# suous/RecNeXt

Measured on AMD Instinct MI355X. Metric: images/sec RecNeXt-M3 224x224 bf16, higher is better.
Workload: dtype bf16

## Files before the change

### recnext_amd/csrc/rcx_mlp.hip

```cpp
#include "rcx_common.h"
#include "rcx_launch.h"
#include "rcx_gelu.h"
#include <type_traits>

#ifdef RCX_MLP_STAMPS
#define RCX_MLP_STAMP(k)                                                                                        \
    {                                                                                                           \
        __builtin_amdgcn_sched_barrier(0);                                                                      \
        unsigned long long t_;                                                                                  \
        asm volatile("s_memtime %0\n\ts_waitcnt lgkmcnt(0)" : "=s"(t_)::"memory");                              \
        __builtin_amdgcn_sched_barrier(0);                                                                      \
        tsum[k] += t_ - tlast;                                                                                  \
        tlast = t_;                                                                                             \
    }
#define RCX_MLP_STAMP_BEGIN                                                                                     \
    unsigned long long tsum[7] = {0, 0, 0, 0, 0, 0, 0}, tlast;                                                  \
    asm volatile("s_memtime %0\n\ts_waitcnt lgkmcnt(0)" : "=s"(tlast)::"memory");
#define RCX_MLP_STAMP_STEP tsum[6] += 1;
#define RCX_MLP_STAMP_END(slot)                                                                                 \
    if (stamps && (threadIdx.x & 63) == 0) {                                                                    \
        _Pragma("unroll") for (int k_ = 0; k_ < 7; ++k_) stamps[(size_t)(slot) * 8 + k_] = tsum[k_];            \
    }
#define RCX_MLP_STAMP_PARM , unsigned long long (&tsum)[7], unsigned long long& tlast
#define RCX_MLP_STAMP_PASS , tsum, tlast
#define RCX_MLP_STAMP_ARG , unsigned long long* __restrict__ stamps
#define RCX_MLP_STAMP_VAL , g_stamps
namespace rcx {
static unsigned long long* g_stamps = nullptr;
}
#else
#define RCX_MLP_STAMP(k)
#define RCX_MLP_STAMP_BEGIN
#define RCX_MLP_STAMP_STEP
#define RCX_MLP_STAMP_END(slot)
#define RCX_MLP_STAMP_PARM
#define RCX_MLP_STAMP_PASS
#define RCX_MLP_STAMP_ARG
#define RCX_MLP_STAMP_VAL
#endif

#ifndef RCX_MLP_PINNED
#define RCX_MLP_PINNED true
#endif

namespace rcx {
namespace mlp {

typedef float f32x16 __attribute__((ext_vector_type(16)));
typedef float f32x4q __attribute__((ext_vector_type(4)));
typedef float f32x2q __attribute__((ext_vector_type(2)));
typedef __bf16 bf16x8 __attribute__((ext_vector_type(8)));
typedef __bf16 bf16x4 __attribute__((ext_vector_type(4)));
typedef unsigned u32x4q __attribute__((ext_vector_type(4)));
typedef unsigned u32x2q __attribute__((ext_vector_type(2)));

__device__ __forceinline__ void wave_sync()
{
    __builtin_amdgcn_fence(__ATOMIC_RELEASE, "wavefront");
    __builtin_amdgcn_wave_barrier();
    __builtin_amdgcn_fence(__ATOMIC_ACQUIRE, "wavefront");
}


__device__ __forceinline__ __amdgpu_buffer_rsrc_t token_rows(const void* p, unsigned nbytes) { return __builtin_amdgcn_make_buffer_rsrc((void*)p, 0, nbytes, 0x00020000); }

#define RCX_MLP_ZERO(D, N)                                                                                                                \
    _Pragma("unroll") for (int n_ = 0; n_ < N; ++n_) _Pragma("unroll") for (int i_ = 0; i_ < 16; ++i_) D[n_][i_] = 0.f;

#define RCX_MLP_STAGE_Z(ZA)                                                                                                               \
    _Pragma("unroll") for (int q = 0; q < ZH; ++q) {                                                                                      \
        _Pragma("unroll") for (int i = 0; i < KH; ++i) *reinterpret_cast<u32x4q*>(Lt + (ZA)) = zq[q * KH + i];                            \
        wave_sync();                                                                                                                      \
        _Pragma("unroll") for (int k = 0; k < KH; ++k)                                                                                    \
            zb[q * KH + k] = __builtin_bit_cast(bf16x8, *reinterpret_cast<const u32x4q*>(Lt + r * ZP + 32 * k + 16 * h));                 \
        wave_sync();                                                                                                                      \
    }

#define RCX_MLP_IMAGE_QUAD(D2, B2, DST)                                                                                                   \
    {                                                                                                                                     \
        const f32x4q bb = *reinterpret_cast<const f32x4q*>(B2);                                                                           \
        *reinterpret_cast<f32x4q*>(DST) = f32x4q{D2[4 * g] + bb.x, D2[4 * g + 1] + bb.y, D2[4 * g + 2] + bb.z, D2[4 * g + 3] + bb.w};     \
    }

__device__ __forceinline__ bf16x8 rows_plus_x(f32x4q lo, f32x4q hi, u32x4q xv)
{
    bf16x8 o;
    o[0] = (__bf16)(lo.x + __uint_as_float(xv.x << 16)); o[1] = (__bf16)(lo.y + __uint_as_float(xv.x & 0xffff0000u));
    o[2] = (__bf16)(lo.z + __uint_as_float(xv.y << 16)); o[3] = (__bf16)(lo.w + __uint_as_float(xv.y & 0xffff0000u));
    o[4] = (__bf16)(hi.x + __uint_as_float(xv.z << 16)); o[5] = (__bf16)(hi.y + __uint_as_float(xv.z & 0xffff0000u));
    o[6] = (__bf16)(hi.z + __uint_as_float(xv.w << 16)); o[7] = (__bf16)(hi.w + __uint_as_float(xv.w & 0xffff0000u));
    return o;
}

constexpr int imax(int a, int b) { return a > b ? a : b; }
constexpr size_t bias_bytes(int HT, int CT) { return sizeof(float) * 32 * (HT + CT); }

template <int KS1, int HT, int CT, int NW, bool STAGED>
struct SmallLds {
    static constexpr int NF = HT * (KS1 + 2 * CT), ZP = 32 * KS1 + 16, OP = 128 * CT + 16, IMG = STAGED ? 32 * imax(ZP, OP) : 0;
    static constexpr size_t b1 = (size_t)NF * 1024, images = b1 + bias_bytes(HT, CT), bytes = images + (size_t)NW * IMG;
};
template <int KS1, int HT, int CT, int NW, int ZH>
struct StreamLds {
    static constexpr int NCH = KS1 + 2 * CT, ZP = 32 * KS1 / ZH + 16, OP = 256 + 16, IMG = 32 * imax(ZP, OP);
    static constexpr size_t b1 = (size_t)2 * NCH * 1024, images = b1 + bias_bytes(HT, CT), bytes = images + (size_t)NW * IMG;
};
template <int KS1, int HT, int CT>
struct PairLds {
    static constexpr int NW = 8, NS = 3, ZH = 4, NCH = KS1 + 2 * CT, ZP = 32 * KS1 / ZH + 16, OP = 128 + 16, IMG = 32 * imax(ZP, OP);
    static constexpr size_t b1 = (size_t)NS * NCH * 1024, images = b1 + bias_bytes(HT, CT), bytes = images + (size_t)NW * IMG;
};
template <int KS1, int HT, int CT>
struct Res128Lds {
    static constexpr int NW = 8, ZH = 4, NCH = KS1 + 2 * CT, NF = HT * NCH, ZP = 32 * KS1 / ZH + 16, OC = 16, OP = 4 * OC + 16, IMG = 32 * imax(ZP, OP);
    static constexpr size_t b1 = (size_t)NF * 1024, images = b1 + bias_bytes(HT, CT), bytes = images + (size_t)NW * IMG;
};
template <int KS1, int HT, int CT, int NW>
struct WideLds {
    static constexpr int ZBYTES = 2 * KS1 * 1024, XBYTES = NW * 4 * 1024, OP = 256 + 16, IMG = 32 * OP;
    static constexpr size_t xchg = ZBYTES, b1 = (size_t)ZBYTES + 2 * XBYTES, bytes = b1 + bias_bytes(HT, CT);
    static_assert(NW * IMG <= ZBYTES + XBYTES, "the output images alias the z fragments and exchange buffer 0");
};

#define RCX_MLP_HIDDEN_GELU(D1, QUAD)                                                                                                     \
    bf16x8 hb[2];                                                                                                                         \
    gelu_f32x2 gv[8];                                                                                                                     \
    _Pragma("unroll") for (int g = 0; g < 4; ++g) {                                                                                       \
        const f32x4q bb = QUAD;                                                                                                           \
        gv[2 * g] = gelu_f32x2{D1[4 * g] + bb.x, D1[4 * g + 1] + bb.y};                                                                   \
        gv[2 * g + 1] = gelu_f32x2{D1[4 * g + 2] + bb.z, D1[4 * g + 3] + bb.w};                                                           \
    }                                                                                                                                     \
    {                                                                                                                                     \
        gelu_f32x2 ga[4] = {gv[0], gv[1], gv[2], gv[3]}, gb[4] = {gv[4], gv[5], gv[6], gv[7]};                                            \
        gelu2x_batch<4>(ga);                                                                                                              \
        gelu2x_batch<4>(gb);                                                                                                              \
        _Pragma("unroll") for (int i = 0; i < 4; ++i) { gv[i] = ga[i]; gv[4 + i] = gb[i]; }                                               \
    }                                                                                                                                     \
    _Pragma("unroll") for (int g = 0; g < 4; ++g) {                                                                                       \
        hb[g >> 1][4 * (g & 1) + 0] = (__bf16)gv[2 * g].x; hb[g >> 1][4 * (g & 1) + 1] = (__bf16)gv[2 * g].y;                             \
        hb[g >> 1][4 * (g & 1) + 2] = (__bf16)gv[2 * g + 1].x; hb[g >> 1][4 * (g & 1) + 3] = (__bf16)gv[2 * g + 1].y;                     \
    }

template <int KS1, int CT, int RD>
__device__ __forceinline__ void hidden_tile_ring(const u32x4q* Lc, const float* b1t, int lane, int h, const bf16x8 (&zb)[KS1], f32x16 (&d2)[CT] RCX_MLP_STAMP_PARM)
{
    constexpr int R1 = KS1 < RD ? KS1 : RD, N2 = 2 * CT, R2 = N2 < RD ? N2 : RD;
    u32x4q ring[RD];
#pragma unroll
    for (int j = 0; j < R1; ++j) ring[j] = Lc[j * 64 + lane];
    RCX_MLP_STAMP(0)
    f32x16 d1;
#pragma unroll
    for (int i = 0; i < 16; ++i) d1[i] = 0.f;
#pragma unroll
    for (int ks = 0; ks < KS1; ++ks) {
        const bf16x8 a = __builtin_bit_cast(bf16x8, ring[ks % R1]);
        if (ks + R1 < KS1) ring[ks % R1] = Lc[(ks + R1) * 64 + lane];
        d1 = __builtin_amdgcn_mfma_f32_32x32x16_bf16(a, zb[ks], d1, 0, 0, 0);
    }
    RCX_MLP_STAMP(1)
#ifndef RCX_MLP_STAMPS
#pragma unroll
    for (int f = 0; f < R2; ++f) ring[f] = Lc[(KS1 + 2 * (f % CT) + f / CT) * 64 + lane];
#endif
    RCX_MLP_HIDDEN_GELU(d1, *reinterpret_cast<const f32x4q*>(b1t + 8 * g + 4 * h))
#ifdef RCX_MLP_STAMPS
#pragma unroll
    for (int f = 0; f < R2; ++f) ring[f] = Lc[(KS1 + 2 * (f % CT) + f / CT) * 64 + lane];
#endif
    RCX_MLP_STAMP(2)
#pragma unroll
    for (int f = 0; f < N2; ++f) {
        const bf16x8 a = __builtin_bit_cast(bf16x8, ring[f % R2]);
        if (f + R2 < N2) ring[f % R2] = Lc[(KS1 + 2 * ((f + R2) % CT) + (f + R2) / CT) * 64 + lane];
        d2[f % CT] = __builtin_amdgcn_mfma_f32_32x32x16_bf16(a, hb[f / CT], d2[f % CT], 0, 0, 0);
    }
    RCX_MLP_STAMP(3)
}

template <int KS1, int CT, int RD, int PRE2, int B1AT>
__device__ __forceinline__ void hidden_tile_pinned(const u32x4q* Lc, const float* b1t, int lane, int h, const bf16x8 (&zb)[KS1], f32x16 (&d2)[CT] RCX_MLP_STAMP_PARM)
{
    constexpr int R1 = KS1 < RD ? KS1 : RD, N2 = 2 * CT, R2 = N2 < RD ? N2 : RD, P2 = PRE2 < R2 ? PRE2 : R2;
    static_assert(B1AT >= 1 && B1AT <= KS1 && P2 >= 1, "b1 is requested inside D1, W2 before the GELU");
    u32x4q ring[RD];
#pragma unroll
    for (int j = 0; j < R1; ++j) ring[j] = Lc[j * 64 + lane];
    RCX_MLP_STAMP(0)
    f32x16 d1;
#pragma unroll
    for (int i = 0; i < 16; ++i) d1[i] = 0.f;
    f32x4q bq[4];
#pragma unroll
    for (int ks = 0; ks < KS1; ++ks) {
        const bf16x8 a = __builtin_bit_cast(bf16x8, ring[ks % R1]);
        if (ks + R1 < KS1) ring[ks % R1] = Lc[(ks + R1) * 64 + lane];
        if (ks == KS1 - B1AT) {
#pragma unroll
            for (int g = 0; g < 4; ++g) bq[g] = *reinterpret_cast<const f32x4q*>(b1t + 8 * g + 4 * h);
        }
        d1 = __builtin_amdgcn_mfma_f32_32x32x16_bf16(a, zb[ks], d1, 0, 0, 0);
        __builtin_amdgcn_sched_barrier(0);
    }
    RCX_MLP_STAMP(1)
#pragma unroll
    for (int f = 0; f < P2; ++f) ring[f] = Lc[(KS1 + 2 * (f % CT) + f / CT) * 64 + lane];
    __builtin_amdgcn_sched_barrier(0);
    RCX_MLP_HIDDEN_GELU(d1, bq[g])
    __builtin_amdgcn_sched_barrier(0);
#pragma unroll
    for (int f = P2; f < R2; ++f) ring[f] = Lc[(KS1 + 2 * (f % CT) + f / CT) * 64 + lane];
    __builtin_amdgcn_sched_barrier(0);
    RCX_MLP_STAMP(2)
#pragma unroll
    for (int f = 0; f < N2; ++f) {
        const bf16x8 a = __builtin_bit_cast(bf16x8, ring[f % R2]);
        if (f + R2 < N2) ring[f % R2] = Lc[(KS1 + 2 * ((f + R2) % CT) + (f + R2) / CT) * 64 + lane];
        d2[f % CT] = __builtin_amdgcn_mfma_f32_32x32x16_bf16(a, hb[f / CT], d2[f % CT], 0, 0, 0);
        __builtin_amdgcn_sched_barrier(0);
    }
    RCX_MLP_STAMP(3)
}

template <int KS1, int HT, int CT, int NW, int WPS, bool KX, bool OX, bool STAGED>
__global__ void __launch_bounds__(64 * NW, WPS)
k_channel_mlp(const bf16_t* __restrict__ z, const bf16_t* __restrict__ xres, bf16_t* __restrict__ y, const u32x4q* __restrict__ wfrag, const float* __restrict__ bias,
              int M, int C, int ntiles RCX_MLP_STAMP_ARG)
{
    extern __shared__ __attribute__((aligned(16))) unsigned char lds_raw[];
    using L = SmallLds<KS1, HT, CT, NW, STAGED>;
    constexpr int NF = L::NF;
    const u32x4q* const Lf = reinterpret_cast<const u32x4q*>(lds_raw);
    const float* const Lb1 = reinterpret_cast<const float*>(lds_raw + L::b1);
    const float* const Lb2 = Lb1 + 32 * HT;
    {
        u32x4q* Lw = reinterpret_cast<u32x4q*>(lds_raw);
        for (int i = threadIdx.x; i < NF * 64; i += 64 * NW) Lw[i] = wfrag[i];
        float* Lb = reinterpret_cast<float*>(lds_raw + L::b1);
        for (int i = threadIdx.x; i < 32 * (HT + CT); i += 64 * NW) Lb[i] = bias[i];
    }
    __syncthreads();
    const int wave = threadIdx.x >> 6, lane = threadIdx.x & 63, r = lane & 31, h = lane >> 5;
    const unsigned nbytes = (unsigned)M * (unsigned)C * 2u;
    const __amdgpu_buffer_rsrc_t zsrc = token_rows(z, nbytes), xsrc = token_rows(xres, nbytes), ysrc = token_rows(y, nbytes);
    unsigned zk[KS1], oc[CT][4];
#pragma unroll
    for (int ks = 0; ks < KS1; ++ks) zk[ks] = KX || 16 * ks + 8 * h < C ? 2u * (16 * ks + 8 * h) : 0x80000000u;
#pragma unroll
    for (int ct = 0; ct < CT; ++ct)
#pragma unroll
        for (int g = 0; g < 4; ++g) oc[ct][g] = OX || 32 * ct + 8 * g + 4 * h < C ? 2u * (32 * ct + 8 * g + 4 * h) : 0x80000000u;

    RCX_MLP_STAMP_BEGIN
    auto hidden_tile = [&](int ht, const bf16x8 (&zb)[KS1], f32x16 (&d2)[CT]) {
        hidden_tile_ring<KS1, CT, 4>(Lf + (size_t)ht * (KS1 + 2 * CT) * 64, Lb1 + 32 * ht, lane, h, zb, d2 RCX_MLP_STAMP_PASS);
        RCX_MLP_STAMP_STEP
    };
    const int stride = gridDim.x * NW;
    int tile = blockIdx.x * NW + wave;
    if constexpr (STAGED) {
        constexpr int ZP = L::ZP, OP = L::OP;
        unsigned char* const Lt = lds_raw + L::images + (size_t)wave * L::IMG;
        const unsigned RB = 2u * (unsigned)C;
        unsigned go[KS1], za[KS1], oa[KS1];
        bool live[KS1];
#pragma unroll
        for (int i = 0; i < KS1; ++i) {
            const unsigned o = 1024u * i + 16u * lane, t = o / RB, bb = o - t * RB;
            live[i] = o < 32u * RB;
            go[i] = live[i] ? o : 0x80000000u;
            za[i] = t * ZP + bb;
            oa[i] = t * OP + 2u * bb;
        }
        u32x4q zq[KS1];
        auto load_z = [&](int t) {
#pragma unroll
            for (int i = 0; i < KS1; ++i) zq[i] = __builtin_bit_cast(u32x4q, __builtin_amdgcn_raw_buffer_load_b128(zsrc, (int)((unsigned)t * 32u * RB + go[i]), 0, 0));
        };
        if (tile < ntiles) load_z(tile);
        for (; tile < ntiles; tile += stride) {
            const unsigned base = (unsigned)tile * 32u * RB;
#pragma unroll
            for (int i = 0; i < KS1; ++i)
                if (live[i]) *reinterpret_cast<u32x4q*>(Lt + za[i]) = zq[i];
            wave_sync();
            bf16x8 zb[KS1];
#pragma unroll
            for (int ks = 0; ks < KS1; ++ks) {
                u32x4q v = *reinterpret_cast<const u32x4q*>(Lt + r * ZP + 32 * ks + 16 * h);
                if (!KX && ks == KS1 - 1 && !(16 * ks + 8 * h < C)) v = u32x4q{0u, 0u, 0u, 0u};
                zb[ks] = __builtin_bit_cast(bf16x8, v);
            }
            wave_sync();
            if (tile + stride < ntiles) load_z(tile + stride);
            u32x4q xq[KS1];
#pragma unroll
            for (int i = 0; i < KS1; ++i) xq[i] = __builtin_bit_cast(u32x4q, __builtin_amdgcn_raw_buffer_load_b128(xsrc, (int)(base + go[i]), 0, 0));
            f32x16 d2[CT];
            RCX_MLP_ZERO(d2, CT)
            RCX_MLP_STAMP(5)
#pragma unroll 1
            for (int ht = 0; ht < HT; ++ht) hidden_tile(ht, zb, d2);
// ... 72 lines not shown
    const __amdgpu_buffer_rsrc_t zsrc = token_rows(z, nbytes), xsrc = token_rows(xres, nbytes), ysrc = token_rows(y, nbytes);
    static_assert(HT % 2 == 0, "the ring alternates two register sets");
    u32x4q cp[2][PER];
    auto request = [&](u32x4q (&dst)[PER], int chunk) {
#pragma unroll
        for (int i = 0; i < PER; ++i)
            if (!RAG || i + 1 < PER || threadIdx.x + i * NT < NCH * 64) dst[i] = wfrag[(size_t)chunk * NCH * 64 + threadIdx.x + i * NT];
    };
    auto deposit = [&](const u32x4q (&src)[PER], int slot) {
        u32x4q* const Ln = Lring + slot * NCH * 64;
#pragma unroll
        for (int i = 0; i < PER; ++i)
            if (!RAG || i + 1 < PER || threadIdx.x + i * NT < NCH * 64) Ln[threadIdx.x + i * NT] = src[i];
    };
    request(cp[0], 0);
    deposit(cp[0], 0);
    request(cp[1], 1 % HT);
    __syncthreads();
    static_assert(CT % 2 == 0, "output in halves of two tiles");
    static_assert(KS1 % ZH == 0, "column parts of whole k-steps");
    constexpr int RB = 32 * KS1, RBH = RB / ZH, KH = KS1 / ZH, ZP = L::ZP, OP = L::OP, NH = CT / 2;
    unsigned char* const Lt = lds_raw + L::images + (size_t)wave * L::IMG;
    unsigned zo[KS1], za[KS1];
#pragma unroll
    for (int i = 0; i < KS1; ++i) {
        const unsigned o = 1024u * (i % KH) + 16u * lane, t = o / RBH, bz = o % RBH;
        zo[i] = t * RB + (i / KH) * RBH + bz;
        za[i] = t * ZP + bz;
    }
    const unsigned ht_tok = lane >> 3, ht_b = 16u * (lane & 7);
    u32x4q zq[KS1];
    auto load_z = [&](int blk) {
        const unsigned base = (unsigned)(32 * (blk * NW + wave)) * (unsigned)RB;
#pragma unroll
        for (int i = 0; i < KS1; ++i) zq[i] = __builtin_bit_cast(u32x4q, __builtin_amdgcn_raw_buffer_load_b128(zsrc, (int)(base + zo[i]), 0, 0));
    };
    if (ZPF && (int)blockIdx.x < nblocks) load_z(blockIdx.x);
    for (int block = blockIdx.x; block < nblocks; block += gridDim.x) {
        const unsigned base = (unsigned)(32 * (block * NW + wave)) * (unsigned)RB;
        if constexpr (!ZPF) load_z(block);
        bf16x8 zb[KS1];
        RCX_MLP_STAGE_Z(za[q * KH + i])
        if (ZPF && block + (int)gridDim.x < nblocks) load_z(block + gridDim.x);
        f32x16 d2[CT];
        RCX_MLP_ZERO(d2, CT)
        u32x4q xq[NH][4];
#pragma unroll 1
        for (int ht = 0; ht < HT; ht += 2) {
            request(cp[0], (ht + 2) % HT);
            if (ht == HT - 2) {
#pragma unroll
                for (int hf = 0; hf < NH; ++hf)
#pragma unroll
                    for (int j = 0; j < 4; ++j)
                        xq[hf][j] = __builtin_bit_cast(u32x4q, __builtin_amdgcn_raw_buffer_load_b128(xsrc, (int)(128u * hf + ht_b < RB ? base + (8u * j + ht_tok) * RB + 128u * hf + ht_b : 0x80000000u), 0, 0));
            }
            hidden_tile_ring<KS1, CT, (NW > 4 || KS1 > 16 ? 4 : 8)>(Lring, Lb1 + 32 * ht, lane, h, zb, d2 RCX_MLP_STAMP_PASS);
            deposit(cp[1], 1);
            __syncthreads();
            request(cp[1], (ht + 3) % HT);
            hidden_tile_ring<KS1, CT, (NW > 4 || KS1 > 16 ? 4 : 8)>(Lring + NCH * 64, Lb1 + 32 * (ht + 1), lane, h, zb, d2 RCX_MLP_STAMP_PASS);
            deposit(cp[0], 0);
            __syncthreads();
        }
#pragma unroll
        for (int hf = 0; hf < NH; ++hf) {
#pragma unroll
            for (int c2 = 0; c2 < 2; ++c2)
#pragma unroll
                for (int g = 0; g < 4; ++g) RCX_MLP_IMAGE_QUAD(d2[2 * hf + c2], Lb2 + 32 * (2 * hf + c2) + 8 * g + 4 * h, Lt + r * OP + 4 * (32 * c2 + 8 * g + 4 * h))
            wave_sync();
#pragma unroll
            for (int j = 0; j < 4; ++j) {
                const unsigned char* src = Lt + (8 * j + ht_tok) * OP + 2 * ht_b;
                const f32x4q lo = *reinterpret_cast<const f32x4q*>(src), hi = *reinterpret_cast<const f32x4q*>(src + 16);
                __builtin_amdgcn_raw_buffer_store_b128(__builtin_bit_cast(u32x4q, rows_plus_x(lo, hi, xq[hf][j])), ysrc, (int)(128u * hf + ht_b < RB ? base + (8u * j + ht_tok) * RB + 128u * hf + ht_b : 0x80000000u), 0, 0);
            }
            wave_sync();
        }
    }
}


template <int KS1, int HT, int CT, bool PIN>
__global__ void __launch_bounds__(512, 2)
k_channel_mlp_pair(const bf16_t* __restrict__ z, const bf16_t* __restrict__ xres, bf16_t* __restrict__ y, const u32x4q* __restrict__ wfrag, const float* __restrict__ bias,
                   int M, int C, int nblocks RCX_MLP_STAMP_ARG)
{
    extern __shared__ __attribute__((aligned(16))) unsigned char lds_raw[];
    using L = PairLds<KS1, HT, CT>;
    constexpr int NW = L::NW, NT = 64 * NW, NS = L::NS, NCH = L::NCH, PER = NCH * 64 / NT;
    static_assert(NCH * 64 % NT == 0 && HT >= 2, "whole pieces per wave");
    constexpr int ZH = L::ZH, RB = 32 * KS1, RBH = RB / ZH, KH = KS1 / ZH, ZP = L::ZP, OP = L::OP;
    static_assert(KS1 % ZH == 0 && RBH == 128, "column parts of 64 channels: a request = 8 token rows of 128 bytes");
    u32x4q* const Lring = reinterpret_cast<u32x4q*>(lds_raw);
    float* const Lb1 = reinterpret_cast<float*>(lds_raw + L::b1);
    const float* const Lb2 = Lb1 + 32 * HT;
    const int wave = threadIdx.x >> 6, lane = threadIdx.x & 63, r = lane & 31, h = lane >> 5;
    const int wv = __builtin_amdgcn_readfirstlane(wave);
    unsigned char* const Lt = lds_raw + L::images + (size_t)wv * L::IMG;
    auto fill = [&](int chunk, int slot) {
        const u32x4q* src = wfrag + (size_t)chunk * NCH * 64 + threadIdx.x;
        u32x4q* dst = Lring + (size_t)slot * NCH * 64 + wv * 64;
        if constexpr (PIN) {
            const unsigned l0 = (unsigned)(size_t)(__attribute__((address_space(3))) void*)dst;
            unsigned m0_;
#pragma unroll
            for (int i = 0; i < PER; ++i)
                asm volatile("s_mov_b32 %0, m0\n\ts_mov_b32 m0, %2\n\ts_nop 0\n\tglobal_load_lds_dwordx4 %1, off\n\ts_mov_b32 m0, %0" : "=&s"(m0_) : "v"(src + i * NT), "s"(l0 + 16u * i * NT) : "memory");
        } else {
#pragma unroll
            for (int i = 0; i < PER; ++i)
                __builtin_amdgcn_global_load_lds((__attribute__((address_space(1))) void*)(src + i * NT), (__attribute__((address_space(3))) void*)(dst + i * NT), 16, 0, 0);
        }
    };
    constexpr int VM_ALL = 0x70, VM_NEXT = 0x70 | (PER & 15) | ((PER >> 4) << 14);
    fill(0, 0);
    fill(1, 1);
    for (int i = threadIdx.x; i < 32 * (HT + CT); i += NT) Lb1[i] = bias[i];
    const unsigned nbytes = (unsigned)M * (unsigned)C * 2u;
    const __amdgpu_buffer_rsrc_t zsrc = token_rows(z, nbytes), xsrc = token_rows(xres, nbytes), ysrc = token_rows(y, nbytes);
    const unsigned zo0 = (unsigned)(lane >> 3) * RB + 16u * (lane & 7), za0 = (unsigned)(lane >> 3) * ZP + 16u * (lane & 7);
    const unsigned ot = lane >> 2, ob = 16u * (lane & 3);
    if (!(__builtin_popcount(wv) & 1)) __builtin_amdgcn_s_setprio(1);
    RCX_MLP_STAMP_BEGIN
    int slot = 0;
    for (int block = blockIdx.x; block < nblocks; block += gridDim.x) {
        const unsigned base = (unsigned)(32 * (block * NW + wave)) * (unsigned)RB;
        const bool more = block + (int)gridDim.x < nblocks;
        bf16x8 zb[KS1];
        {
            u32x4q zq[KS1];
#pragma unroll
            for (int i = 0; i < KS1; ++i)
                zq[i] = __builtin_bit_cast(u32x4q, __builtin_amdgcn_raw_buffer_load_b128(zsrc, (int)(base + zo0 + 8u * RB * (i % KH) + RBH * (i / KH)), 0, 0));
            RCX_MLP_STAGE_Z(za0 + 8 * ZP * i)
        }
        f32x16 d2[CT];
        RCX_MLP_ZERO(d2, CT)
        RCX_MLP_STAMP(5)
#pragma unroll 1
        for (int ht = 0; ht < HT; ++ht) {
            if (ht + 1 < HT || more) __builtin_amdgcn_s_waitcnt(VM_NEXT);
            else __builtin_amdgcn_s_waitcnt(VM_ALL);
            __builtin_amdgcn_s_barrier();
            if (ht + 2 < HT || more) fill((ht + 2) % HT, slot == 0 ? 2 : slot - 1);
            RCX_MLP_STAMP(4)
            if constexpr (PIN) {
                hidden_tile_pinned<KS1, CT, 4, 1, 3>(Lring + (size_t)slot * NCH * 64, Lb1 + 32 * ht, lane, h, zb, d2 RCX_MLP_STAMP_PASS);
            } else
                hidden_tile_ring<KS1, CT, 4>(Lring + (size_t)slot * NCH * 64, Lb1 + 32 * ht, lane, h, zb, d2 RCX_MLP_STAMP_PASS);
            RCX_MLP_STAMP_STEP
            slot = slot == NS - 1 ? 0 : slot + 1;
        }
        u32x4q xq[CT][2];
#pragma unroll
        for (int ct = 0; ct < CT; ++ct)
#pragma unroll
            for (int j = 0; j < 2; ++j)
                xq[ct][j] = __builtin_bit_cast(u32x4q, __builtin_amdgcn_raw_buffer_load_b128(xsrc, (int)(base + (16u * j + ot) * RB + 64u * ct + ob), 0, 0));
#pragma unroll
        for (int ct = 0; ct < CT; ++ct) {
#pragma unroll
            for (int g = 0; g < 4; ++g) RCX_MLP_IMAGE_QUAD(d2[ct], Lb2 + 32 * ct + 8 * g + 4 * h, Lt + r * OP + 4 * (8 * g + 4 * h))
            wave_sync();
#pragma unroll
            for (int j = 0; j < 2; ++j) {
                const unsigned char* src = Lt + (16 * j + ot) * OP + 2 * ob;
                const f32x4q lo = *reinterpret_cast<const f32x4q*>(src), hi = *reinterpret_cast<const f32x4q*>(src + 16);
                __builtin_amdgcn_raw_buffer_store_b128(__builtin_bit_cast(u32x4q, rows_plus_x(lo, hi, xq[ct][j])), ysrc, (int)(base + (16u * j + ot) * RB + 64u * ct + ob), 0, 0);
            }
            wave_sync();
        }
    }
    RCX_MLP_STAMP(5)
    RCX_MLP_STAMP_END(blockIdx.x * NW + wv)
}


template <int KS1, int HT, int CT>
__global__ void __launch_bounds__(512, 2)
k_channel_mlp_res128(const bf16_t* __restrict__ z, const bf16_t* __restrict__ xres, bf16_t* __restrict__ y, const u32x4q* __restrict__ wfrag, const float* __restrict__ bias,
                     int M, int ntiles RCX_MLP_STAMP_ARG)
{
    extern __shared__ __attribute__((aligned(16))) unsigned char lds_raw[];
    using L = Res128Lds<KS1, HT, CT>;
    constexpr int NW = L::NW, NT = 64 * NW, NCH = L::NCH, NF = L::NF, PER = NF * 64 / NT;
    static_assert(NF * 64 % NT == 0, "whole pieces per wave");
    constexpr int ZH = L::ZH, RB = 32 * KS1, RBH = RB / ZH, KH = KS1 / ZH, ZP = L::ZP;
    static_assert(KS1 % ZH == 0 && RBH == 64, "column parts of 32 channels: a request = 16 token rows of 64 bytes");
    constexpr int OC = L::OC, NP = 32 * CT / OC, OP = L::OP;
    const u32x4q* const Lf = reinterpret_cast<const u32x4q*>(lds_raw);
    float* const Lb1 = reinterpret_cast<float*>(lds_raw + L::b1);
    const float* const Lb2 = Lb1 + 32 * HT;
    const int lane = threadIdx.x & 63, r = lane & 31, h = lane >> 5;
    const int wv = __builtin_amdgcn_readfirstlane(threadIdx.x >> 6);
    unsigned char* const Lt = lds_raw + L::images + (size_t)wv * L::IMG;
    {
        const u32x4q* src = wfrag + threadIdx.x;
        u32x4q* dst = reinterpret_cast<u32x4q*>(lds_raw) + wv * 64;
#pragma unroll
        for (int i = 0; i < PER; ++i)
            __builtin_amdgcn_global_load_lds((__attribute__((address_space(1))) void*)(src + i * NT), (__attribute__((address_space(3))) void*)(dst + i * NT), 16, 0, 0);
        for (int i = threadIdx.x; i < 32 * (HT + CT); i += NT) Lb1[i] = bias[i];
    }
    const unsigned nbytes = (unsigned)M * (unsigned)RB;
    const __amdgpu_buffer_rsrc_t zsrc = token_rows(z, nbytes), xsrc = token_rows(xres, nbytes), ysrc = token_rows(y, nbytes);
    const unsigned zo0 = (unsigned)(lane >> 2) * RB + 16u * (lane & 3), za0 = (unsigned)(lane >> 2) * ZP + 16u * (lane & 3);
    const unsigned ot = lane / 2, ob = 16u * (lane % 2);
    const int stride = NW * (int)gridDim.x;
    int tile = wv * (int)gridDim.x + (int)blockIdx.x;
    u32x4q zq[KS1];
    auto load_z = [&](int t) {
        const unsigned base = (unsigned)t * 32u * RB;
#pragma unroll
        for (int i = 0; i < KS1; ++i)
            zq[i] = __builtin_bit_cast(u32x4q, __builtin_amdgcn_raw_buffer_load_b128(zsrc, (int)(base + zo0 + 16u * RB * (i % KH) + RBH * (i / KH)), 0, 0));
    };
    if (tile < ntiles) load_z(tile);
    __builtin_amdgcn_s_waitcnt(0x70);
    __syncthreads();
    RCX_MLP_STAMP_BEGIN
    for (; tile < ntiles; tile += stride) {
        const unsigned base = (unsigned)tile * 32u * RB;
        bf16x8 zb[KS1];
        RCX_MLP_STAGE_Z(za0 + 16 * ZP * i)
        if (tile + stride < ntiles) load_z(tile + stride);
        f32x16 d2[CT];
        RCX_MLP_ZERO(d2, CT)
        RCX_MLP_STAMP(5)
#pragma unroll 1
        for (int ht = 0; ht < HT; ++ht) {
            hidden_tile_ring<KS1, CT, 4>(Lf + (size_t)ht * NCH * 64, Lb1 + 32 * ht, lane, h, zb, d2 RCX_MLP_STAMP_PASS);
            RCX_MLP_STAMP_STEP
        }
        u32x4q xq[NP];
#pragma unroll
        for (int p = 0; p < NP; ++p) xq[p] = __builtin_bit_cast(u32x4q, __builtin_amdgcn_raw_buffer_load_b128(xsrc, (int)(base + ot * RB + 2u * OC * p + ob), 0, 0));
#pragma unroll
        for (int p = 0; p < NP; ++p) {
#pragma unroll
            for (int g = 2 * (p & 1); g < 2 * (p & 1) + 2; ++g) RCX_MLP_IMAGE_QUAD(d2[p >> 1], Lb2 + 32 * (p >> 1) + 8 * g + 4 * h, Lt + r * OP + 4 * (8 * (g & 1) + 4 * h))
            wave_sync();
            const unsigned char* src = Lt + ot * OP + 2 * ob;
            const f32x4q lo = *reinterpret_cast<const f32x4q*>(src), hi = *reinterpret_cast<const f32x4q*>(src + 16);
            __builtin_amdgcn_raw_buffer_store_b128(__builtin_bit_cast(u32x4q, rows_plus_x(lo, hi, xq[p])), ysrc, (int)(base + ot * RB + 2u * OC * p + ob), 0, 0);
            wave_sync();
        }
    }
    RCX_MLP_STAMP(5)
    RCX_MLP_STAMP_END(wv * (int)gridDim.x + (int)blockIdx.x)
}


template <int KS1, int HT, int CT, int RD, int NW = 8>
__global__ void __launch_bounds__(64 * NW, 2)
k_channel_mlp_wide(const bf16_t* __restrict__ z, const bf16_t* __restrict__ xres, bf16_t* __restrict__ y, const u32x4q* __restrict__ wfrag, const float* __restrict__ bias, int M)
{
    extern __shared__ __attribute__((aligned(16))) unsigned char lds_raw[];
// ... 115 lines not shown
    step(NST - 1, std::true_type{});
    unsigned char* const Lt = lds_raw + (size_t)wv * L::IMG;
#pragma unroll
    for (int tt = 0; tt < 2; ++tt) {
#pragma unroll
        for (int c2 = 0; c2 < 2; ++c2)
#pragma unroll
            for (int g = 0; g < 4; ++g) RCX_MLP_IMAGE_QUAD(d2[c2][tt], Lb2 + 32 * (2 * wv + c2) + 8 * g + 4 * h, Lt + r * OP + 4 * (32 * c2 + 8 * g + 4 * h))
        wave_sync();
#pragma unroll
        for (int j = 0; j < 4; ++j) {
            const unsigned char* src = Lt + (8 * j + ot) * OP + 2 * ob;
            const f32x4q lo = *reinterpret_cast<const f32x4q*>(src), hi = *reinterpret_cast<const f32x4q*>(src + 16);
            __builtin_amdgcn_raw_buffer_store_b128(__builtin_bit_cast(u32x4q, rows_plus_x(lo, hi, xq[tt][j])), ysrc, (int)(base + (32u * tt + 8u * j + ot) * RB + 128u * wv + ob), 0, 0);
        }
        wave_sync();
    }
}

}

constexpr int mlp_ks1(int C) { return (C + 15) / 16; }
constexpr int mlp_ct(int C) { return C > 128 ? (C + 63) / 64 * 2 : (C + 31) / 32; }

static bool mlp_shape(int C, int H, int* ks1, int* ht, int* ct)
{
    if (C <= 0 || H <= 0 || C % 8 || H % 32) return false;
    *ks1 = mlp_ks1(C); *ht = H / 32; *ct = mlp_ct(C);
    return true;
}

size_t channel_mlp_pack_bytes(int C, int H)
{
    int ks1, ht, ct;
    if (!mlp_shape(C, H, &ks1, &ht, &ct)) return 0;
    return (size_t)(ht * ks1 + ct * 2 * ht) * 1024;
}

#define RCX_MLP_LAUNCH_ARGS const void* z, const void* x, void* y, const void* wfrag, const float* bias, int M, int C, int ncu, hipStream_t s
typedef hipError_t (*mlp_launcher)(RCX_MLP_LAUNCH_ARGS);

template <int CH, int HT>
static hipError_t launch_mlp(RCX_MLP_LAUNCH_ARGS)
{
    constexpr int KS1 = mlp_ks1(CH), CT = mlp_ct(CH);
    constexpr int NW = CT <= 2 ? 12 : 8, WPS = NW / 4;
    constexpr bool STAGED = CT <= 2;
    using L = mlp::SmallLds<KS1, HT, CT, NW, STAGED>;
    static_assert(L::bytes <= 160 * 1024, "weights + the waves' images must fit the LDS");
    if (C != CH) return hipErrorInvalidConfiguration;
    auto kfn = mlp::k_channel_mlp<KS1, HT, CT, NW, WPS, CH == 16 * KS1, CH == 32 * CT, STAGED>;
    RCX_SET_LDS_ONCE(kfn, L::bytes);
    const int ntiles = (M + 31) / 32;
    int grid = ncu;
    if (grid * NW > ntiles) grid = (ntiles + NW - 1) / NW;
    hipLaunchKernelGGL(kfn, dim3((unsigned)grid), dim3(64 * NW), L::bytes, s, (const bf16_t*)z, (const bf16_t*)x, (bf16_t*)y, (const mlp::u32x4q*)wfrag, bias, M, C, ntiles RCX_MLP_STAMP_VAL);
    return hipGetLastError();
}

template <int CH, int HT, int ZH = 1, bool ZPF = true>
static hipError_t launch_mlp_stream(RCX_MLP_LAUNCH_ARGS)
{
    constexpr int KS1 = mlp_ks1(CH), CT = mlp_ct(CH), NW = 4;
    using L = mlp::StreamLds<KS1, HT, CT, NW, ZH>;
    static_assert(L::bytes <= 160 * 1024, "the ring and the waves' images must fit the LDS");
    static_assert(CH == 16 * KS1, "no padding lanes");
    if (C != CH) return hipErrorInvalidConfiguration;
    auto kfn = mlp::k_channel_mlp_stream<KS1, HT, CT, NW, NW / 4, ZH, ZPF>;
    RCX_SET_LDS_ONCE(kfn, L::bytes);
    const int nblocks = (M + 32 * NW - 1) / (32 * NW);
    const int grid = nblocks < ncu ? nblocks : ncu;
    hipLaunchKernelGGL(kfn, dim3((unsigned)grid), dim3(64 * NW), L::bytes, s, (const bf16_t*)z, (const bf16_t*)x, (bf16_t*)y, (const mlp::u32x4q*)wfrag, bias, M, C, nblocks);
    return hipGetLastError();
}

template <int CH, int HT>
static hipError_t launch_mlp_pair(RCX_MLP_LAUNCH_ARGS)
{
    constexpr int KS1 = mlp_ks1(CH), CT = mlp_ct(CH);
    using L = mlp::PairLds<KS1, HT, CT>;
    static_assert(L::bytes <= 160 * 1024, "the ring and the waves' images must fit the LDS");
    static_assert(CH == 16 * KS1, "no padding lanes");
    if (C != CH) return hipErrorInvalidConfiguration;
    auto kfn = mlp::k_channel_mlp_pair<KS1, HT, CT, RCX_MLP_PINNED>;
    RCX_SET_LDS_ONCE(kfn, L::bytes);
    const int nblocks = (M + 32 * L::NW - 1) / (32 * L::NW);
    const int grid = nblocks < ncu ? nblocks : ncu;
    hipLaunchKernelGGL(kfn, dim3((unsigned)grid), dim3(64 * L::NW), L::bytes, s, (const bf16_t*)z, (const bf16_t*)x, (bf16_t*)y, (const mlp::u32x4q*)wfrag, bias, M, C, nblocks RCX_MLP_STAMP_VAL);
    return hipGetLastError();
}

template <int CH, int HT>
static hipError_t launch_mlp_res128(RCX_MLP_LAUNCH_ARGS)
{
    constexpr int KS1 = mlp_ks1(CH), CT = mlp_ct(CH);
    using L = mlp::Res128Lds<KS1, HT, CT>;
    static_assert(L::bytes <= 160 * 1024, "the pack, the biases and the waves' images must fit the LDS");
    static_assert(CH == 16 * KS1, "no padding lanes");
    if (C != CH) return hipErrorInvalidConfiguration;
    auto kfn = mlp::k_channel_mlp_res128<KS1, HT, CT>;
    RCX_SET_LDS_ONCE(kfn, L::bytes);
    const int ntiles = (M + 31) / 32;
    int grid = (ntiles + L::NW - 1) / L::NW;
    if (grid > ncu) grid = ncu;
    hipLaunchKernelGGL(kfn, dim3((unsigned)grid), dim3(64 * L::NW), L::bytes, s, (const bf16_t*)z, (const bf16_t*)x, (bf16_t*)y, (const mlp::u32x4q*)wfrag, bias, M, ntiles RCX_MLP_STAMP_VAL);
    return hipGetLastError();
}

template <int CH, int HT>
static hipError_t launch_mlp_wide(RCX_MLP_LAUNCH_ARGS)
{
    constexpr int KS1 = mlp_ks1(CH), CT = mlp_ct(CH), NW = CT / 2;
    using L = mlp::WideLds<KS1, HT, CT, NW>;
    static_assert(L::bytes <= 160 * 1024, "the z fragments, the exchange buffers and the biases must fit the LDS");
    static_assert(CH == 16 * KS1, "no padding lanes");
    if (C != CH) return hipErrorInvalidConfiguration;
    auto kfn = mlp::k_channel_mlp_wide<KS1, HT, CT, 8, NW>;
    RCX_SET_LDS_ONCE(kfn, L::bytes);
    hipLaunchKernelGGL(kfn, dim3((unsigned)((M + 63) / 64)), dim3(64 * NW), L::bytes, s, (const bf16_t*)z, (const bf16_t*)x, (bf16_t*)y, (const mlp::u32x4q*)wfrag, bias, M);
    return hipGetLastError();
}

struct MlpRow { int C, HT, min_tokens; mlp_launcher launch; };
static constexpr MlpRow MLP_ROWS[] = {
    {256, 16, 1, launch_mlp_pair<256, 16>},
    {128, 8, 1, launch_mlp_res128<128, 8>},
    {512, 32, 2048, launch_mlp_wide<512, 32>},
    {512, 24, 512, launch_mlp_wide<512, 24>},
    {384, 24, 784, launch_mlp_wide<384, 24>},
    {192, 12, 1, launch_mlp_stream<192, 12>},
    {160, 10, 1, launch_mlp_stream<160, 10>},
    {320, 20, 1, launch_mlp_stream<320, 20, 2, false>},
    {64, 4, 1, launch_mlp<64, 4>},
    {56, 4, 1, launch_mlp<56, 4>},
    {48, 3, 1, launch_mlp<48, 3>},
    {40, 3, 1, launch_mlp<40, 3>},
    {96, 6, 1, launch_mlp<96, 6>},
    {80, 5, 1, launch_mlp<80, 5>},
};

static const MlpRow* mlp_row(int M, int C, int H, int dtype)
{
    if (dtype != 1 || M <= 0 || H <= 0 || H % 32) return nullptr;
    if ((unsigned long long)M * C * 2 >= (1ull << 31)) return nullptr;
    for (const MlpRow& row : MLP_ROWS)
        if (row.C == C && row.HT == H / 32) return M >= row.min_tokens ? &row : nullptr;
    return nullptr;
}

bool channel_mlp_applicable(int M, int C, int H, int dtype) { return mlp_row(M, C, H, dtype) != nullptr; }

hipError_t channel_mlp(const void* z, const void* x, void* y, const void* wfrag, const float* bias, int M, int C, int H, int dtype, hipStream_t s)
{
    const MlpRow* const row = mlp_row(M, C, H, dtype);
    if (!row) return hipErrorInvalidConfiguration;
    static std::atomic<int> cus[RCX_MAX_DEVICES];
    int dev = 0, ncu = 256;
    if (hipGetDevice(&dev) == hipSuccess && dev >= 0 && dev < RCX_MAX_DEVICES) {
        ncu = cus[dev].load(std::memory_order_relaxed);
        if (ncu <= 0) {
            int v = 0;
            ncu = hipDeviceGetAttribute(&v, hipDeviceAttributeMultiprocessorCount, dev) == hipSuccess && v > 0 ? v : 256;
            cus[dev].store(ncu, std::memory_order_relaxed);
        }
    }
    return row->launch(z, x, y, wfrag, bias, M, C, ncu, s);
}
// ... 11 lines not shown
```

Measured before the change: 130,400.

## Skew follower waves by half a hidden tile in the pair channel-MLP kernel

Splits the weight ring into separate W1 and W2 slot rings, with three W1 slots and four W2 slots. Half the waves (the followers) run a skewed schedule: each interval does the previous tile's D2 chained into the current tile's D1 and GELU, so that MFMA-heavy and VALU-heavy phases of the two wave halves interleave on the SIMD. The old alternating s_setprio scheme is dropped by default, and lane indices are recomputed to relieve register pressure. The cost is more LDS for the extra W2 slot and more complex control flow with larger code.

```diff
diff --git a/recnext_amd/csrc/rcx_mlp.hip b/recnext_amd/csrc/rcx_mlp.hip
--- a/recnext_amd/csrc/rcx_mlp.hip
+++ b/recnext_amd/csrc/rcx_mlp.hip
@@ -39,8 +39,11 @@
 #define RCX_MLP_STAMP_VAL
 #endif
 
-#ifndef RCX_MLP_PINNED
-#define RCX_MLP_PINNED true
+#ifndef RCX_MLP_SKEW
+#define RCX_MLP_SKEW 2
+#endif
+#ifndef RCX_MLP_SKEW_PRIO
+#define RCX_MLP_SKEW_PRIO (RCX_MLP_SKEW ? 0 : 3)
 #endif
 
 namespace rcx {
@@ -53,6 +56,13 @@
 typedef __bf16 bf16x4 __attribute__((ext_vector_type(4)));
 typedef unsigned u32x4q __attribute__((ext_vector_type(4)));
 typedef unsigned u32x2q __attribute__((ext_vector_type(2)));
+
+__device__ __forceinline__ int lane_again()
+{
+    int l;
+    asm volatile("v_mbcnt_lo_u32_b32 %0, -1, 0\n\tv_mbcnt_hi_u32_b32 %0, -1, %0" : "=v"(l));
+    return l;
+}
 
 __device__ __forceinline__ void wave_sync()
 {
@@ -107,8 +117,8 @@
 };
 template <int KS1, int HT, int CT>
 struct PairLds {
-    static constexpr int NW = 8, NS = 3, ZH = 4, NCH = KS1 + 2 * CT, ZP = 32 * KS1 / ZH + 16, OP = 128 + 16, IMG = 32 * imax(ZP, OP);
-    static constexpr size_t b1 = (size_t)NS * NCH * 1024, images = b1 + bias_bytes(HT, CT), bytes = images + (size_t)NW * IMG;
+    static constexpr int NW = 8, NS1 = 3, NS2 = 4, ZH = 4, NCH = KS1 + 2 * CT, ZP = 32 * KS1 / ZH + 16, OP = 128 + 16, IMG = 32 * imax(ZP, OP);
+    static constexpr size_t w2 = (size_t)NS1 * KS1 * 1024, b1 = w2 + (size_t)NS2 * 2 * CT * 1024, images = b1 + bias_bytes(HT, CT), bytes = images + (size_t)NW * IMG;
 };
 template <int KS1, int HT, int CT>
 struct Res128Lds {
@@ -178,46 +188,59 @@
     RCX_MLP_STAMP(3)
 }
 
-template <int KS1, int CT, int RD, int PRE2, int B1AT>
-__device__ __forceinline__ void hidden_tile_pinned(const u32x4q* Lc, const float* b1t, int lane, int h, const bf16x8 (&zb)[KS1], f32x16 (&d2)[CT] RCX_MLP_STAMP_PARM)
-{
-    constexpr int R1 = KS1 < RD ? KS1 : RD, N2 = 2 * CT, R2 = N2 < RD ? N2 : RD, P2 = PRE2 < R2 ? PRE2 : R2;
-    static_assert(B1AT >= 1 && B1AT <= KS1 && P2 >= 1, "b1 is requested inside D1, W2 before the GELU");
-    u32x4q ring[RD];
-#pragma unroll
-    for (int j = 0; j < R1; ++j) ring[j] = Lc[j * 64 + lane];
-    RCX_MLP_STAMP(0)
-    f32x16 d1;
+#define RCX_MLP_PIN1(ACC)                                                                                                                 \
+    asm volatile("" : "+v"(ACC)::"memory");                                                                                               \
+    __builtin_amdgcn_sched_barrier(0);
+#define RCX_MLP_PIN2(ACC, B0, B1)                                                                                                         \
+    asm volatile("" : "+v"(ACC), "+v"(B0), "+v"(B1)::"memory");                                                                           \
+    __builtin_amdgcn_sched_barrier(0);
+
+template <int KS1, int RD, int B1AT, bool LOADED>
+__device__ __forceinline__ void pinned_d1(const u32x4q* L1, const float* b1t, int lane, int h, const bf16x8 (&zb)[KS1], u32x4q (&ring)[RD], f32x16& d1, f32x4q (&bq)[4] RCX_MLP_STAMP_PARM)
+{
+    constexpr int R1 = KS1 < RD ? KS1 : RD;
+    static_assert(B1AT >= 0 && B1AT <= KS1, "b1 is requested inside D1 or by the caller");
+    if constexpr (!LOADED) {
+#pragma unroll
+        for (int j = 0; j < R1; ++j) ring[j] = L1[j * 64 + lane];
+        RCX_MLP_STAMP(0)
+    }
 #pragma unroll
     for (int i = 0; i < 16; ++i) d1[i] = 0.f;
-    f32x4q bq[4];
 #pragma unroll
     for (int ks = 0; ks < KS1; ++ks) {
         const bf16x8 a = __builtin_bit_cast(bf16x8, ring[ks % R1]);
-        if (ks + R1 < KS1) ring[ks % R1] = Lc[(ks + R1) * 64 + lane];
-        if (ks == KS1 - B1AT) {
+        if (ks + R1 < KS1) ring[ks % R1] = L1[(ks + R1) * 64 + lane];
+        if (B1AT && ks == KS1 - B1AT) {
 #pragma unroll
             for (int g = 0; g < 4; ++g) bq[g] = *reinterpret_cast<const f32x4q*>(b1t + 8 * g + 4 * h);
         }
         d1 = __builtin_amdgcn_mfma_f32_32x32x16_bf16(a, zb[ks], d1, 0, 0, 0);
-        __builtin_amdgcn_sched_barrier(0);
+        RCX_MLP_PIN1(d1)
     }
     RCX_MLP_STAMP(1)
-#pragma unroll
-    for (int f = 0; f < P2; ++f) ring[f] = Lc[(KS1 + 2 * (f % CT) + f / CT) * 64 + lane];
+}
+
+template <int CT, int RD, int FROM, int TO>
+__device__ __forceinline__ void pinned_w2_request(const u32x4q* L2, int lane, u32x4q (&ring)[RD])
+{
+#pragma unroll
+    for (int f = FROM; f < TO; ++f) ring[f] = L2[(2 * (f % CT) + f / CT) * 64 + lane];
     __builtin_amdgcn_sched_barrier(0);
-    RCX_MLP_HIDDEN_GELU(d1, bq[g])
-    __builtin_amdgcn_sched_barrier(0);
-#pragma unroll
-    for (int f = P2; f < R2; ++f) ring[f] = Lc[(KS1 + 2 * (f % CT) + f / CT) * 64 + lane];
-    __builtin_amdgcn_sched_barrier(0);
-    RCX_MLP_STAMP(2)
+}
+
+template <int KS1, int CT, int RD, bool CHAIN>
+__device__ __forceinline__ void pinned_d2(const u32x4q* L2, const u32x4q* L1n, int lane, bf16x8 (&hb)[2], u32x4q (&ring)[RD], f32x16 (&d2)[CT] RCX_MLP_STAMP_PARM)
+{
+    constexpr int R1 = KS1 < RD ? KS1 : RD, N2 = 2 * CT, R2 = N2 < RD ? N2 : RD;
+    static_assert(!CHAIN || (R1 == R2 && N2 % R2 == 0), "the chained D1 finds fragment j in ring[j % R1]");
 #pragma unroll
     for (int f = 0; f < N2; ++f) {
         const bf16x8 a = __builtin_bit_cast(bf16x8, ring[f % R2]);
-        if (f + R2 < N2) ring[f % R2] = Lc[(KS1 + 2 * ((f + R2) % CT) + (f + R2) / CT) * 64 + lane];
+        if (f + R2 < N2) ring[f % R2] = L2[(2 * ((f + R2) % CT) + (f + R2) / CT) * 64 + lane];
+        else if (CHAIN) ring[f % R2] = L1n[(f + R2 - N2) * 64 + lane];
         d2[f % CT] = __builtin_amdgcn_mfma_f32_32x32x16_bf16(a, hb[f / CT], d2[f % CT], 0, 0, 0);
-        __builtin_amdgcn_sched_barrier(0);
+        RCX_MLP_PIN2(d2[f % CT], hb[0], hb[1])
     }
     RCX_MLP_STAMP(3)
 }
@@ -456,54 +479,108 @@
 }
 
 
-template <int KS1, int HT, int CT, bool PIN>
+#define RCX_MLP_PAIR_INTERVALS(HEAD, STEP, TAIL)                                                                                          \
+    {                                                                                                                                     \
+        open_interval(0);                                                                                                                 \
+        HEAD                                                                                                                              \
+        _Pragma("unroll 1") for (int s = 1; s < HT; ++s) {                                                                                \
+            open_interval(s);                                                                                                             \
+            STEP                                                                                                                          \
+        }                                                                                                                                 \
+        last_interval();                                                                                                                  \
+        TAIL                                                                                                                              \
+    }
+
+#define RCX_MLP_PAIR_GELU                                                                                                                 \
+        {                                                                                                                                 \
+            RCX_MLP_HIDDEN_GELU(d1, bq[g])                                                                                                \
+            hk[0] = hb[0];                                                                                                                \
+            hk[1] = hb[1];                                                                                                                \
+        }                                                                                                                                 \
+        __builtin_amdgcn_sched_barrier(0);
+#define RCX_MLP_PAIR_B1(P)                                                                                                                \
+        _Pragma("unroll") for (int g = 0; g < 4; ++g) bq[g] = *reinterpret_cast<const f32x4q*>((P) + 8 * g + 4 * h);
+#define RCX_MLP_PAIR_LEAD                                                                                                                 \
+        pinned_d1<KS1, 4, 3, false>(W1c, b1c, lane, h, zb, ring, d1, bq RCX_MLP_STAMP_PASS);                                              \
+        pinned_w2_request<CT, 4, 0, 1>(W2c, lane, ring);                                                                                  \
+        RCX_MLP_PAIR_GELU                                                                                                                 \
+        pinned_w2_request<CT, 4, 1, 4>(W2c, lane, ring);                                                                                  \
+        RCX_MLP_STAMP(2)                                                                                                                  \
+        pinned_d2<KS1, CT, 4, false>(W2c, W1c, lane, hk, ring, d2 RCX_MLP_STAMP_PASS);                                                    \
+        RCX_MLP_STAMP_STEP
+#define RCX_MLP_PAIR_NONE
+#define RCX_MLP_PAIR_B_D1G(LOADED)                                                                                                        \
+        pinned_d1<KS1, 4, 3, LOADED>(W1c, b1c, lane, h, zb, ring, d1, bq RCX_MLP_STAMP_PASS);                                             \
+        RCX_MLP_PAIR_GELU                                                                                                                 \
+        RCX_MLP_STAMP(2)                                                                                                                  \
+        RCX_MLP_STAMP_STEP
+#define RCX_MLP_PAIR_B_D2(CHAIN)                                                                                                          \
+        pinned_w2_request<CT, 4, 0, 4>(W2p, lane, ring);                                                                                  \
+        RCX_MLP_STAMP(0)                                                                                                                  \
+        pinned_d2<KS1, CT, 4, CHAIN>(W2p, W1c, lane, hk, ring, d2 RCX_MLP_STAMP_PASS);
+#define RCX_MLP_PAIR_B_HEAD RCX_MLP_PAIR_B_D1G(false)
+#define RCX_MLP_PAIR_B_STEP RCX_MLP_PAIR_B_D2(true) RCX_MLP_PAIR_B_D1G(true)
+#define RCX_MLP_PAIR_B_TAIL RCX_MLP_PAIR_B_D2(false)
+#define RCX_MLP_PAIR_A_GD2(B1P, CHAIN)                                                                                                    \
+        RCX_MLP_PAIR_B1(B1P)                                                                                                              \
+        pinned_w2_request<CT, 4, 0, 1>(W2p, lane, ring);                                                                                  \
+        RCX_MLP_PAIR_GELU                                                                                                                 \
+        pinned_w2_request<CT, 4, 1, 4>(W2p, lane, ring);                                                                                  \
+        RCX_MLP_STAMP(2)                                                                                                                  \
+        pinned_d2<KS1, CT, 4, CHAIN>(W2p, W1c, lane, hk, ring, d2 RCX_MLP_STAMP_PASS);                                                    \
+        RCX_MLP_STAMP_STEP
+#define RCX_MLP_PAIR_A_HEAD pinned_d1<KS1, 4, 0, false>(W1c, b1c, lane, h, zb, ring, d1, bq RCX_MLP_STAMP_PASS);
+#define RCX_MLP_PAIR_A_STEP RCX_MLP_PAIR_A_GD2(b1c - 32, true) pinned_d1<KS1, 4, 0, true>(W1c, b1c, lane, h, zb, ring, d1, bq RCX_MLP_STAMP_PASS);
+#define RCX_MLP_PAIR_A_TAIL RCX_MLP_PAIR_A_GD2(Lb1 + 32 * (HT - 1), false)
+
+template <int KS1, int HT, int CT, int SKEW>
 __global__ void __launch_bounds__(512, 2)
 k_channel_mlp_pair(const bf16_t* __restrict__ z, const bf16_t* __restrict__ xres, bf16_t* __restrict__ y, const u32x4q* __restrict__ wfrag, const float* __restrict__ bias,
                    int M, int C, int nblocks RCX_MLP_STAMP_ARG)
 {
     extern __shared__ __attribute__((aligned(16))) unsigned char lds_raw[];
     using L = PairLds<KS1, HT, CT>;
-    constexpr int NW = L::NW, NT = 64 * NW, NS = L::NS, NCH = L::NCH, PER = NCH * 64 / NT;
+    constexpr int NW = L::NW, NT = 64 * NW, NS1 = L::NS1, NS2 = L::NS2, NCH = L::NCH, N2 = 2 * CT, PER = NCH * 64 / NT;
     static_assert(NCH * 64 % NT == 0 && HT >= 2, "whole pieces per wave");
+    static_assert(KS1 % NW == 0, "a wave's piece i (fragment NW i + w of the chunk) lies in the W1 half for NW i < KS1 and in the W2 half from there, whatever the wave");
+    static_assert(NS1 >= 3 && NS2 >= 4, "the slot rule: chunks n .. n + 2 of W1 and n - 1 .. n + 2 of W2 are in distinct slots");
     constexpr int ZH = L::ZH, RB = 32 * KS1, RBH = RB / ZH, KH = KS1 / ZH, ZP = L::ZP, OP = L::OP;
     static_assert(KS1 % ZH == 0 && RBH == 128, "column parts of 64 channels: a request = 8 token rows of 128 bytes");
-    u32x4q* const Lring = reinterpret_cast<u32x4q*>(lds_raw);
+    u32x4q* const Lw1 = reinterpret_cast<u32x4q*>(lds_raw);
+    u32x4q* const Lw2 = reinterpret_cast<u32x4q*>(lds_raw + L::w2);
     float* const Lb1 = reinterpret_cast<float*>(lds_raw + L::b1);
     const float* const Lb2 = Lb1 + 32 * HT;
-    const int wave = threadIdx.x >> 6, lane = threadIdx.x & 63, r = lane & 31, h = lane >> 5;
+    const int wave = threadIdx.x >> 6, lane = threadIdx.x & 63, h = lane >> 5;
     const int wv = __builtin_amdgcn_readfirstlane(wave);
     unsigned char* const Lt = lds_raw + L::images + (size_t)wv * L::IMG;
-    auto fill = [&](int chunk, int slot) {
+    auto fill = [&](int chunk, int slot1, int slot2) {
         const u32x4q* src = wfrag + (size_t)chunk * NCH * 64 + threadIdx.x;
-        u32x4q* dst = Lring + (size_t)slot * NCH * 64 + wv * 64;
-        if constexpr (PIN) {
-            const unsigned l0 = (unsigned)(size_t)(__attribute__((address_space(3))) void*)dst;
-            unsigned m0_;
-#pragma unroll
-            for (int i = 0; i < PER; ++i)
-                asm volatile("s_mov_b32 %0, m0\n\ts_mov_b32 m0, %2\n\ts_nop 0\n\tglobal_load_lds_dwordx4 %1, off\n\ts_mov_b32 m0, %0" : "=&s"(m0_) : "v"(src + i * NT), "s"(l0 + 16u * i * NT) : "memory");
-        } else {
-#pragma unroll
-            for (int i = 0; i < PER; ++i)
-                __builtin_amdgcn_global_load_lds((__attribute__((address_space(1))) void*)(src + i * NT), (__attribute__((address_space(3))) void*)(dst + i * NT), 16, 0, 0);
-        }
+        const unsigned l1 = (unsigned)(size_t)(__attribute__((address_space(3))) void*)(Lw1 + (size_t)slot1 * KS1 * 64 + wv * 64);
+        const unsigned l2 = (unsigned)(size_t)(__attribute__((address_space(3))) void*)(Lw2 + (size_t)slot2 * N2 * 64 + wv * 64);
+        unsigned m0_;
+#pragma unroll
+        for (int i = 0; i < PER; ++i)
+            asm volatile("s_mov_b32 %0, m0\n\ts_mov_b32 m0, %2\n\ts_nop 0\n\tglobal_load_lds_dwordx4 %1, off\n\ts_mov_b32 m0, %0"
+                         : "=&s"(m0_) : "v"(src + i * NT), "s"(NW * i < KS1 ? l1 + 16u * i * NT : l2 + 16u * (i * NT - KS1 * 64)) : "memory");
     };
     constexpr int VM_ALL = 0x70, VM_NEXT = 0x70 | (PER & 15) | ((PER >> 4) << 14);
-    fill(0, 0);
-    fill(1, 1);
+    fill(0, 0, 0);
+    fill(1, 1, 1);
     for (int i = threadIdx.x; i < 32 * (HT + CT); i += NT) Lb1[i] = bias[i];
     const unsigned nbytes = (unsigned)M * (unsigned)C * 2u;
     const __amdgpu_buffer_rsrc_t zsrc = token_rows(z, nbytes), xsrc = token_rows(xres, nbytes), ysrc = token_rows(y, nbytes);
-    const unsigned zo0 = (unsigned)(lane >> 3) * RB + 16u * (lane & 7), za0 = (unsigned)(lane >> 3) * ZP + 16u * (lane & 7);
-    const unsigned ot = lane >> 2, ob = 16u * (lane & 3);
-    if (!(__builtin_popcount(wv) & 1)) __builtin_amdgcn_s_setprio(1);
+    const bool follower = SKEW != 0 && wv >= NW / 2;
+    if (RCX_MLP_SKEW_PRIO == 3 ? !(__builtin_popcount(wv) & 1) : RCX_MLP_SKEW_PRIO == 2 ? wv >= NW / 2 : RCX_MLP_SKEW_PRIO == 1 ? wv < NW / 2 : false)
+        __builtin_amdgcn_s_setprio(1);
     RCX_MLP_STAMP_BEGIN
-    int slot = 0;
+    int c1 = 0, c2 = 0;
     for (int block = blockIdx.x; block < nblocks; block += gridDim.x) {
-        const unsigned base = (unsigned)(32 * (block * NW + wave)) * (unsigned)RB;
+        const unsigned base = (unsigned)(32 * (block * NW + wv)) * (unsigned)RB;
         const bool more = block + (int)gridDim.x < nblocks;
         bf16x8 zb[KS1];
         {
+            const int lz = lane_again(), r = lz & 31, h = lz >> 5;
+            const unsigned zo0 = (unsigned)(lz >> 3) * RB + 16u * (lz & 7), za0 = (unsigned)(lz >> 3) * ZP + 16u * (lz & 7);
             u32x4q zq[KS1];
 #pragma unroll
             for (int i = 0; i < KS1; ++i)
@@ -513,20 +590,35 @@
         f32x16 d2[CT];
         RCX_MLP_ZERO(d2, CT)
         RCX_MLP_STAMP(5)
-#pragma unroll 1
-        for (int ht = 0; ht < HT; ++ht) {
-            if (ht + 1 < HT || more) __builtin_amdgcn_s_waitcnt(VM_NEXT);
+        const u32x4q *W1c, *W2c, *W2p;
+        const float* b1c;
+        auto open_interval = [&](int s) {
+            if (s + 1 < HT || more) __builtin_amdgcn_s_waitcnt(VM_NEXT);
             else __builtin_amdgcn_s_waitcnt(VM_ALL);
             __builtin_amdgcn_s_barrier();
-            if (ht + 2 < HT || more) fill((ht + 2) % HT, slot == 0 ? 2 : slot - 1);
+            if (s + 2 < HT || more) fill((s + 2) % HT, c1 == 0 ? NS1 - 1 : c1 - 1, (c2 + 2) % NS2);
             RCX_MLP_STAMP(4)
-            if constexpr (PIN) {
-                hidden_tile_pinned<KS1, CT, 4, 1, 3>(Lring + (size_t)slot * NCH * 64, Lb1 + 32 * ht, lane, h, zb, d2 RCX_MLP_STAMP_PASS);
-            } else
-                hidden_tile_ring<KS1, CT, 4>(Lring + (size_t)slot * NCH * 64, Lb1 + 32 * ht, lane, h, zb, d2 RCX_MLP_STAMP_PASS);
-            RCX_MLP_STAMP_STEP
-            slot = slot == NS - 1 ? 0 : slot + 1;
-        }
+            W1c = Lw1 + (size_t)c1 * KS1 * 64;
+            W2c = Lw2 + (size_t)c2 * N2 * 64;
+            W2p = Lw2 + (size_t)((c2 + NS2 - 1) % NS2) * N2 * 64;
+            b1c = Lb1 + 32 * s;
+            c1 = c1 == NS1 - 1 ? 0 : c1 + 1;
+            c2 = (c2 + 1) % NS2;
+        };
+        auto last_interval = [&]() {
+            __builtin_amdgcn_s_barrier();
+            RCX_MLP_STAMP(4)
+            W2p = Lw2 + (size_t)((c2 + NS2 - 1) % NS2) * N2 * 64;
+        };
+        u32x4q ring[4];
+        f32x16 d1;
+        f32x4q bq[4];
+        bf16x8 hk[2];
+        if (!follower) RCX_MLP_PAIR_INTERVALS(RCX_MLP_PAIR_LEAD, RCX_MLP_PAIR_LEAD, RCX_MLP_PAIR_NONE)
+        else if constexpr (SKEW == 2) RCX_MLP_PAIR_INTERVALS(RCX_MLP_PAIR_B_HEAD, RCX_MLP_PAIR_B_STEP, RCX_MLP_PAIR_B_TAIL)
+        else RCX_MLP_PAIR_INTERVALS(RCX_MLP_PAIR_A_HEAD, RCX_MLP_PAIR_A_STEP, RCX_MLP_PAIR_A_TAIL)
+        const int le = lane_again(), r = le & 31, h = le >> 5;
+        const unsigned ot = le >> 2, ob = 16u * (le & 3);
         u32x4q xq[CT][2];
 #pragma unroll
         for (int ct = 0; ct < CT; ++ct)
@@ -549,6 +641,9 @@
     }
     RCX_MLP_STAMP(5)
     RCX_MLP_STAMP_END(blockIdx.x * NW + wv)
+#ifdef RCX_MLP_STAMPS
+    if (stamps && lane == 0) stamps[(size_t)(blockIdx.x * NW + wv) * 8 + 7] = (unsigned long long)__builtin_amdgcn_s_getreg(4 | (0 << 6) | (31 << 11));
+#endif
 }
 
 
@@ -830,7 +925,7 @@
     static_assert(L::bytes <= 160 * 1024, "the ring and the waves' images must fit the LDS");
     static_assert(CH == 16 * KS1, "no padding lanes");
     if (C != CH) return hipErrorInvalidConfiguration;
-    auto kfn = mlp::k_channel_mlp_pair<KS1, HT, CT, RCX_MLP_PINNED>;
+    auto kfn = mlp::k_channel_mlp_pair<KS1, HT, CT, RCX_MLP_SKEW>;
     RCX_SET_LDS_ONCE(kfn, L::bytes);
     const int nblocks = (M + 32 * L::NW - 1) / (32 * L::NW);
     const int grid = nblocks < ncu ? nblocks : ncu;
```

New measurement: 130,200. Within noise of the previous version (-0.1%).
